# ooowedyn/InkLayer

Hardware: AMD Instinct MI355X
Metric: sketches/sec end-to-end (GroundingDINO+SAM) at 1024x1024 (higher is better)
Workload: dtype f16 (MFMA, f32 accumulate; f32 residual/norm/softmax; split-f16 = fp32-grade operands for patch-embed, neck, mask decoder)

## Files before the change

include/inklayer_hip.h:

```cpp
#ifndef INKLAYER_HIP_H
#define INKLAYER_HIP_H

#include <stdint.h>

#ifdef __cplusplus
extern "C" {
#endif

#define INK_ABI_VERSION 7
int ink_abi_version(void);

typedef struct InkGemm {
  const void* A;
  const void* W;
  const float* bias;
  const float* col_scale;
  const float* residual;
  const int32_t* row_map;
  void* C;
  int32_t M, N, K;
  int32_t lda, ldw, ldr, ldc;
  int32_t act;
  int32_t c_f16;
} InkGemm;
// ... 111 lines not shown

int ink_biattn_fusion(const void* QV_f16, const void* KL_f16, int32_t B, int32_t S, int32_t T, int32_t E,
                      float scale, float* scores_ws, float* stats_ws, float* partial_ws, int32_t chunk,
                      void* out_v_f16, void* out_l_f16, void* stream);

int ink_attn_fewkeys(const void* Q, int64_t ldq, const void* K, int64_t ldk, const void* V, int64_t ldv,
                     int32_t B, int32_t n_q, int32_t n_k, int32_t n_heads, int32_t head_dim, float scale,
                     const uint8_t* blocked, const int32_t* q_batch_rows, const float* q_add, int32_t io_f32, void* O,
                     int64_t ldo, void* stream);

int ink_attn_fewq(const void* Q, int64_t ldq, const void* K, int64_t ldk, const void* V, int64_t ldv,
                  int32_t n_batch, int32_t n_q, int32_t n_k, int32_t n_heads, int32_t head_dim, float scale,
                  const int32_t* q_batch_rows, const int32_t* kv_batch_rows, const float* k_add, int32_t io_f32, void* O,
                  int64_t ldo, void* stream);

int ink_biattn_colstats(const float* scores, int32_t B, int32_t S, int32_t HT, float* part_ws, float* stats, void* stream);

int ink_fusion_fold_workspace(int32_t B, int32_t S, int64_t* out_floats);
int ink_fusion_fold(float* v_f32, int32_t B, int32_t S, const float* lnv_g, const float* lnv_b, float eps,
                    const float* text_k_f32, const float* text_vl_f32, int64_t ld_text, int32_t T, const void* Wq_f16,
                    const float* bq, const void* Wvv_f16, const float* bvv, const void* Wo_f16, const float* bo,
                    const float* gamma_v, float scale, float* ws, void* out_l_f16, const float* pos, void* out16_pos,
                    void* out16, void* stream);

int ink_sam_upscale_pack(const void* ws_f16, void* blob_f16, void* stream);
int ink_sam_upscale_tail(const float* u0, int64_t ld_tok, int32_t n, int32_t g, const float* ln_g, const float* ln_b, float eps,
                         const void* blob_f16, const float* b3, const float* hyper, int32_t n_masks, float* low,
                         void* stream);

int ink_proj256_ln_pack(const void* ws_f16, void* blob_f16, void* stream);
int ink_proj256_ln(const float* a_f32, const void* blob_f16, const float* bias, const float* res_f32,
                   const int32_t* res_batch_rows, int32_t rows_per_batch, const float* ln_g, const float* ln_b, float eps,
                   int64_t rows, float* out_f32, void* out_split_f16, void* stream);

int ink_ffn256_pack_bytes(int32_t hid, int32_t with_pre, int64_t* out_bytes);
int ink_ffn256_pack(const void* w1_f16, const float* b1, const void* w2_f16, int32_t hid, const void* wpre_f16, void* blob,
                    void* stream);
int ink_ffn256_fused(const void* x_f16, int64_t ldx, const float* res_f32, const void* blob, const float* b2,
                     const float* ln_g, const float* ln_b, float eps, int32_t M, int32_t hid, const float* pre_bias,
                     const float* pre_ln_g, const float* pre_ln_b, float* out_f32, void* stream);

int ink_topk_rowmax(const float* logits, int32_t B, int32_t S, int32_t T, int32_t K, int32_t* out_idx,
                    float* out_val, void* cand_ws, void* stream);

int ink_sine_embed4(const float* ref, const float* dim_t, int32_t N, void* out_f16, void* stream);

int ink_box_refine(const float* delta, int64_t ldd, const float* ref, int32_t N, int32_t ref_is_logit,
                   float* out, void* stream);

int ink_mask_cleanup_workspace_ints(int32_t n, int32_t H, int32_t W, int32_t k, int64_t* out_ints);
int ink_mask_cleanup(const void* masks_u8, int32_t n, int32_t H, int32_t W, int32_t k, int32_t area_threshold,
                     double aspect_threshold, void* tmp_a_u8, void* tmp_b_u8, int32_t* workspace, void* out_u8,
                     void* stream);

int ink_mask_sketch_iou_counts(const void* masks_u8, const void* sketch_rgb_u8, int32_t n, int32_t H, int32_t W,
                               void* bits_ws_u64, int32_t* counts, void* stream);

int ink_sam_amg_stats(const float* low, int32_t n, const int32_t* index, int32_t m, const int32_t* m_dev, int32_t S,
                      int32_t L, int32_t in_h, int32_t in_w, int32_t crop_h, int32_t crop_w, double thr, double offset,
                      int32_t x0, int32_t y0, int32_t orig_h, int32_t orig_w, int32_t* table, void* planes_u64,
                      float* out_logits, void* stream);

int ink_mask_rle_counts(const void* planes_u64, const int32_t* select, int32_t k, int32_t H, int32_t W,
                        int32_t* n_counts, void* stream);
int ink_mask_rle_write(const void* planes_u64, const int32_t* select, int32_t k, int32_t H, int32_t W,
                       const int32_t* offsets, int32_t* counts, void* stream);
// ... 54 lines not shown
```

inklayer_amd/_lib.py:

```python
from __future__ import annotations

import ctypes as C
import os
from pathlib import Path

_LIB_PATH = Path(__file__).resolve().parent / "lib" / "libinklayer_hip.so"
_lib = None

c_void_p, c_int, c_i64, c_float = C.c_void_p, C.c_int32, C.c_int64, C.c_float


class InkGemm(C.Structure):
    _fields_ = [
        ("A", c_void_p), ("W", c_void_p), ("bias", c_void_p), ("col_scale", c_void_p),
        ("residual", c_void_p), ("row_map", c_void_p), ("C", c_void_p),
        ("M", c_int), ("N", c_int), ("K", c_int),
        ("lda", c_int), ("ldw", c_int), ("ldr", c_int), ("ldc", c_int),
        ("act", c_int), ("c_f16", c_int),
    ]


class InkAttn(C.Structure):
    _fields_ = [
        ("Q", c_void_p), ("K", c_void_p), ("V", c_void_p), ("O", c_void_p),
# ... 33 lines not shown
                            c_void_p, c_void_p, c_void_p],
    "ink_sam_amg_stats": [c_void_p, c_int, c_void_p, c_int, c_void_p, c_int, c_int, c_int, c_int, c_int, c_int, C.c_double,
                          C.c_double, c_int, c_int, c_int, c_int, c_void_p, c_void_p, c_void_p, c_void_p],
    "ink_mask_rle_counts": [c_void_p, c_void_p, c_int, c_int, c_int, c_void_p, c_void_p],
    "ink_mask_rle_write": [c_void_p, c_void_p, c_int, c_int, c_int, c_void_p, c_void_p, c_void_p],
    "ink_mask_small_regions_workspace_ints": [c_int, c_int, c_int, C.POINTER(c_i64)],
    "ink_mask_small_regions": [c_void_p, c_int, c_int, c_int, c_int, c_int, c_void_p, c_void_p, c_void_p, c_void_p,
                               c_void_p],
    "ink_box_nms": [c_void_p, c_void_p, c_int, c_float, c_void_p, c_void_p, c_void_p, c_void_p],
    "ink_ms_deform_attn_forward": [c_void_p, C.POINTER(c_i64), C.POINTER(c_i64), c_void_p, c_void_p, c_int,
                                   c_int, c_int, c_int, c_int, c_int, c_int, c_int, c_void_p, c_void_p],
    "ink_ms_deform_attn_forward_dev": [c_void_p, c_void_p, c_void_p, c_void_p, c_void_p, c_int, c_int, c_int, c_int,
                                       c_int, c_int, c_int, c_int, c_int, c_void_p, c_void_p],
    "ink_ms_deform_attn_backward_dev": [c_void_p, c_void_p, c_void_p, c_void_p, c_void_p, c_void_p, c_int, c_int, c_int,
                                        c_int, c_int, c_int, c_int, c_int, c_int, c_void_p, c_void_p, c_void_p,
                                        c_void_p],
    "ink_msda_fused": [c_void_p, c_void_p, c_i64, c_void_p, c_int, c_i64, c_i64, C.POINTER(c_int), c_int,
                       c_int, c_int, c_void_p, c_void_p],
    "ink_swin_patchify": [c_void_p, c_int, c_int, C.POINTER(c_float), C.POINTER(c_float), c_void_p, c_void_p],
    "ink_layernorm_merge4": [c_void_p, c_i64, c_void_p, c_void_p, c_float, c_void_p, c_int, c_int, c_void_p,
                             c_void_p],
    "ink_groupnorm_nhwc": [c_void_p, c_int, c_int, c_int, c_int, c_void_p, c_void_p, c_float, c_void_p,
                           c_void_p, c_i64, c_void_p],
    "ink_gather_rows": [c_void_p, c_i64, c_i64, c_void_p, c_i64, c_int, c_int, c_int, c_void_p, c_void_p,
                        c_void_p],
    "ink_biattn_fusion": [c_void_p, c_void_p, c_int, c_int, c_int, c_int, c_float, c_void_p, c_void_p,
                          c_void_p, c_int, c_void_p, c_void_p, c_void_p],
    "ink_biattn_colstats": [c_void_p, c_int, c_int, c_int, c_void_p, c_void_p, c_void_p],
    "ink_fusion_fold_workspace": [c_int, c_int, C.POINTER(c_i64)],
    "ink_relpos_bias64_f16": [c_void_p, c_i64, c_void_p, c_void_p, c_int, c_int, c_int, c_float, c_void_p, c_void_p, c_void_p],
    "ink_proj256_ln_pack": [c_void_p, c_void_p, c_void_p],
    "ink_proj256_ln": [c_void_p, c_void_p, c_void_p, c_void_p, c_void_p, c_int, c_void_p, c_void_p, c_float, c_i64, c_void_p,
                       c_void_p, c_void_p],
    "ink_sam_upscale_pack": [c_void_p, c_void_p, c_void_p],
    "ink_sam_upscale_tail": [c_void_p, c_i64, c_int, c_int, c_void_p, c_void_p, c_float, c_void_p, c_void_p, c_void_p,
                             c_int, c_void_p, c_void_p],
    "ink_ffn256_pack_bytes": [c_int, c_int, C.POINTER(c_i64)],
    "ink_ffn256_pack": [c_void_p, c_void_p, c_void_p, c_int, c_void_p, c_void_p, c_void_p],
    "ink_ffn256_fused": [c_void_p, c_i64, c_void_p, c_void_p, c_void_p, c_void_p, c_void_p, c_float, c_int, c_int,
                         c_void_p, c_void_p, c_void_p, c_void_p, c_void_p],
    "ink_fusion_fold": [c_void_p, c_int, c_int, c_void_p, c_void_p, c_float, c_void_p, c_void_p, c_i64, c_int, c_void_p,
                        c_void_p, c_void_p, c_void_p, c_void_p, c_void_p, c_void_p, c_float, c_void_p, c_void_p, c_void_p,
                        c_void_p, c_void_p, c_void_p],
    "ink_attn_fewkeys": [c_void_p, c_i64, c_void_p, c_i64, c_void_p, c_i64, c_int, c_int, c_int, c_int, c_int,
                         c_float, c_void_p, c_void_p, c_void_p, c_int, c_void_p, c_i64, c_void_p],
    "ink_attn_fewq": [c_void_p, c_i64, c_void_p, c_i64, c_void_p, c_i64, c_int, c_int, c_int, c_int, c_int,
                      c_float, c_void_p, c_void_p, c_void_p, c_int, c_void_p, c_i64, c_void_p],
    "ink_topk_rowmax": [c_void_p, c_int, c_int, c_int, c_int, c_void_p, c_void_p, c_void_p, c_void_p],
    "ink_sine_embed4": [c_void_p, c_void_p, c_int, c_void_p, c_void_p],
    "ink_box_refine": [c_void_p, c_i64, c_void_p, c_int, c_int, c_void_p, c_void_p],
    "ink_mask_cleanup_workspace_ints": [c_int, c_int, c_int, c_int, C.POINTER(c_i64)],
    "ink_mask_cleanup": [c_void_p, c_int, c_int, c_int, c_int, c_int, C.c_double, c_void_p, c_void_p, c_void_p,
                         c_void_p, c_void_p],
    "ink_mask_sketch_iou_counts": [c_void_p, c_void_p, c_int, c_int, c_int, c_void_p, c_void_p, c_void_p],
    "ink_refine_sketch_planes": [c_void_p, c_int, c_int, c_void_p, c_void_p, c_void_p],
    "ink_bitplane_pack": [c_void_p, c_int, c_int, c_int, c_int, c_void_p, c_void_p],
    "ink_refine_depth_samples": [c_void_p, c_int, c_void_p, c_void_p, c_int, c_int, c_int, c_void_p, c_void_p, c_void_p],
    "ink_refine_pair_tables": [c_void_p, c_void_p, c_int, c_int, c_int, c_void_p, c_void_p, c_void_p, c_void_p,
                               c_void_p, c_void_p],
    "ink_refine_composite": [c_void_p, c_void_p, c_int, c_int, c_int, c_void_p, c_void_p, c_void_p],
    "ink_refine_relabel_clean": [c_void_p, c_void_p, c_int, c_int, c_void_p, c_void_p],
    "ink_refine_grow_workspace": [c_int, c_int, C.POINTER(c_i64), C.POINTER(c_i64)],
    "ink_refine_grow": [c_void_p, c_void_p, c_int, c_int, c_void_p, c_void_p, c_void_p, c_void_p, c_void_p, c_void_p,
                        c_int, c_void_p, c_void_p],
    "ink_refine_query_dists": [c_void_p, c_void_p, c_void_p, c_int, c_int, c_int, c_void_p, c_void_p],
    "ink_refine_finalize": [c_void_p, c_void_p, c_int, c_void_p, c_int, c_int, c_void_p, c_void_p, c_void_p, c_void_p],
# ... 44 lines not shown
```

inklayer_amd/csrc/proj_ln.hip:

```cpp
#include <type_traits>
#include "common.h"
#include "../../include/inklayer_hip.h"

namespace {

typedef __attribute__((address_space(1))) const void* gptr_t;
typedef __attribute__((address_space(3))) void* lptr_t;
typedef __attribute__((address_space(3))) char* lds_char_ptr;

constexpr int CI = 128, C = 256, BM = 128;
constexpr int BLK = 1024;
constexpr int NSEG = 3, KSEG = CI / 16;
constexpr int NBLK = (C / 32) * KSEG;
constexpr int CHUNK = NBLK * BLK;
constexpr int PAR_BYTES = 3 * C * 4;
constexpr int OROW = C * 4 + 16;
constexpr int PAR_OFF = 4 * 32 * OROW;
constexpr int LDS_BYTES = PAR_OFF + PAR_BYTES;
constexpr int DEPTH = 4;
static_assert(PAR_OFF >= 2 * CHUNK && LDS_BYTES <= 160 * 1024, "LDS layout");

template <int I> using ic = std::integral_constant<int, I>;
template <int I, int N, class F>
__device__ __forceinline__ void static_for(F&& f) {
  if constexpr (I < N) {
    f(ic<I>{});
    static_for<I + 1, N>(f);
  }
}
__device__ __forceinline__ f32x16 mfma32(const f16x8& a, const f16x8& b, const f32x16& c) {
  return __builtin_amdgcn_mfma_f32_32x32x16_f16(a, b, c, 0, 0, 0);
}
template <int OFF>
__device__ __forceinline__ f16x8 lds_frag(uint32_t addr) {
  f16x8 v;
  asm volatile("ds_read_b128 %0, %1 offset:%2" : "=v"(v) : "v"(addr), "n"(OFF));
  return v;
}
template <int N>
__device__ __forceinline__ void wait_frag(f16x8& f) {
  asm volatile("s_waitcnt lgkmcnt(%1)" : "+v"(f) : "n"(N));
}
template <int OFF>
__device__ __forceinline__ f32x4 lds_f4(uint32_t addr) {
  f32x4 v;
  asm volatile("ds_read_b128 %0, %1 offset:%2" : "=v"(v) : "v"(addr), "n"(OFF));
  return v;
}
__device__ __forceinline__ void wait_f4(f32x4& a, f32x4& b, f32x4& c, f32x4& d) {
  asm volatile("s_waitcnt lgkmcnt(0)" : "+v"(a), "+v"(b), "+v"(c), "+v"(d));
}

__global__ __launch_bounds__(256) void proj_ln_pack_kernel(const f16* __restrict__ ws, f16* __restrict__ blob) {
  const int idx = blockIdx.x * 256 + threadIdx.x;
  if (idx >= NSEG * NBLK * 64) return;
  const int lane = idx & 63, q = (idx >> 6) % NBLK, seg = (idx >> 6) / NBLK;
  const int nt = q / KSEG, s = KSEG * seg + q % KSEG;
  *(f16x8*)(blob + (int64_t)idx * 8) = *(const f16x8*)(ws + (int64_t)(32 * nt + (lane & 31)) * (NSEG * CI) + 16 * s + 8 * (lane >> 5));
}

__global__ __launch_bounds__(256) void proj256_ln_kernel(const float* __restrict__ A, const f16* __restrict__ blob,
                                                         const float* __restrict__ bias, const float* __restrict__ res,
                                                         const int32_t* __restrict__ res_batch_rows, int rows_per_batch,
                                                         const float* __restrict__ ln_g, const float* __restrict__ ln_b,
                                                         float eps, int64_t R, float* __restrict__ out_f32,
                                                         f16* __restrict__ out_split) {
  extern __shared__ __attribute__((aligned(16))) char smem[];
  const int tid = threadIdx.x, lane = tid & 63;
  const int wave = __builtin_amdgcn_readfirstlane(tid >> 6);
  const int l = lane & 31, hh = lane >> 5;
  const int64_t m0 = (int64_t)blockIdx.x * BM + wave * 32;
  const int64_t row = min(m0 + l, R - 1);
  {
    float* sP = (float*)(smem + PAR_OFF);
    sP[tid] = bias[tid];
    sP[C + tid] = ln_g[tid];
    sP[2 * C + tid] = ln_b[tid];
  }
  f16x8 xf[NSEG * KSEG];
  {
    const float* ap = A + row * CI + 8 * hh;
#pragma unroll
    for (int s = 0; s < KSEG; ++s) {
      const f32x4 a0 = *(const f32x4*)(ap + 16 * s), a1 = *(const f32x4*)(ap + 16 * s + 4);
#pragma unroll
      for (int e = 0; e < 8; ++e) {
        const float v = e < 4 ? a0[e] : a1[e - 4];
        const f16 hi = (f16)v;
        xf[s][e] = hi;
        xf[KSEG + s][e] = (f16)((v - (float)hi) * 64.0f);
        xf[2 * KSEG + s][e] = (f16)((float)hi * 0.015625f);
      }
    }
  }
  f32x16 y[C / 32];
  {
    int64_t rrow = row;
    if (res_batch_rows) {
      const int64_t b = row / rows_per_batch;
      rrow = (int64_t)res_batch_rows[b] + (row - b * rows_per_batch);
    }
    const float* rp = res + rrow * C + 4 * hh;
#pragma unroll
    for (int nt = 0; nt < C / 32; ++nt)
#pragma unroll
      for (int g = 0; g < 4; ++g) {
        const f32x4 r4 = *(const f32x4*)(rp + 32 * nt + 8 * g);
#pragma unroll
        for (int e = 0; e < 4; ++e) y[nt][4 * g + e] = r4[e];
      }
// ... 34 lines not shown

  static_for<0, C / 32>([&](auto ii) {
    constexpr int nt = decltype(ii)::value;
    constexpr int ob = (32 * nt) * 4;
    f32x4 c0 = lds_f4<ob>(par0), c1 = lds_f4<ob + 32>(par0), c2 = lds_f4<ob + 64>(par0), c3 = lds_f4<ob + 96>(par0);
    wait_f4(c0, c1, c2, c3);
#pragma unroll
    for (int e = 0; e < 4; ++e) {
      y[nt][e] += c0[e];
      y[nt][4 + e] += c1[e];
      y[nt][8 + e] += c2[e];
      y[nt][12 + e] += c3[e];
    }
  });
  float sum = 0.f;
#pragma unroll
  for (int nt = 0; nt < C / 32; ++nt)
#pragma unroll
    for (int r = 0; r < 16; ++r) sum += y[nt][r];
  sum += __shfl_xor(sum, 32, 64);
  const float mean = sum * (1.0f / C);
  float sq = 0.f;
#pragma unroll
  for (int nt = 0; nt < C / 32; ++nt)
#pragma unroll
    for (int r = 0; r < 16; ++r) {
      const float d = y[nt][r] - mean;
      sq += d * d;
    }
  sq += __shfl_xor(sq, 32, 64);
  const float rstd = 1.0f / sqrtf(sq * (1.0f / C) + eps);
  __syncthreads();
  char* ot = smem + wave * 32 * OROW;
  static_for<0, C / 32 * 2>([&](auto ii) {
    constexpr int nt = decltype(ii)::value / 2, g = 2 * (decltype(ii)::value % 2);
    constexpr int o0 = C * 4 + (32 * nt + 8 * g) * 4;
    f32x4 g0 = lds_f4<o0>(par0), g1 = lds_f4<o0 + 32>(par0), b0 = lds_f4<C * 4 + o0>(par0), b1 = lds_f4<C * 4 + o0 + 32>(par0);
    wait_f4(g0, g1, b0, b1);
    f32x4 v0, v1;
#pragma unroll
    for (int e = 0; e < 4; ++e) {
      v0[e] = (y[nt][4 * g + e] - mean) * rstd * g0[e] + b0[e];
      v1[e] = (y[nt][4 * g + 4 + e] - mean) * rstd * g1[e] + b1[e];
    }
    *(f32x4*)(ot + l * OROW + (32 * nt + 8 * g + 4 * hh) * 4) = v0;
    *(f32x4*)(ot + l * OROW + (32 * nt + 8 * g + 8 + 4 * hh) * 4) = v1;
  });
#pragma unroll 2
  for (int r = 0; r < 32; ++r) {
    const int64_t m = m0 + r;
    if (m >= R) break;
    const f32x4 v = *(const f32x4*)(ot + r * OROW + lane * 16);
    if (out_f32) *(f32x4*)(out_f32 + m * C + lane * 4) = v;
    if (out_split) {
      f16x4 hi, lo, hs;
#pragma unroll
      for (int e = 0; e < 4; ++e) {
        hi[e] = (f16)v[e];
        lo[e] = (f16)((v[e] - (float)hi[e]) * 64.0f);
        hs[e] = (f16)((float)hi[e] * 0.015625f);
      }
      f16* o = out_split + m * (3 * C) + lane * 4;
      *(f16x4*)o = hi;
      *(f16x4*)(o + C) = lo;
      *(f16x4*)(o + 2 * C) = hs;
    }
  }
}

}

extern "C" int ink_proj256_ln_pack(const void* ws_f16, void* blob_f16, void* stream) {
  INK_CHECK_ARG(ws_f16 && blob_f16 && ((((uintptr_t)ws_f16 | (uintptr_t)blob_f16) & 15) == 0));
  hipLaunchKernelGGL(proj_ln_pack_kernel, dim3((NSEG * NBLK * 64 + 255) / 256), dim3(256), 0, (hipStream_t)stream,
                     (const f16*)ws_f16, (f16*)blob_f16);
  return ink_launch_status();
}

extern "C" int ink_proj256_ln(const float* a_f32, const void* blob_f16, const float* bias, const float* res_f32,
                              const int32_t* res_batch_rows, int32_t rows_per_batch, const float* ln_g, const float* ln_b,
                              float eps, int64_t rows, float* out_f32, void* out_split_f16, void* stream) {
  INK_CHECK_ARG(a_f32 && blob_f16 && bias && res_f32 && ln_g && ln_b && rows > 0 && (out_f32 || out_split_f16));
  INK_CHECK_ARG(!res_batch_rows || (rows_per_batch > 0 && rows % rows_per_batch == 0));
  INK_CHECK_ARG((((uintptr_t)a_f32 | (uintptr_t)blob_f16 | (uintptr_t)res_f32 | (uintptr_t)out_f32 |
                  (uintptr_t)out_split_f16) & 15) == 0);
  static bool attr = ((void)hipFuncSetAttribute((const void*)proj256_ln_kernel, hipFuncAttributeMaxDynamicSharedMemorySize,
                                                LDS_BYTES), true);
  (void)attr;
  const int64_t ntiles = (rows + BM - 1) / BM;
  INK_CHECK_ARG(ntiles < (int64_t)1 << 31);
  hipLaunchKernelGGL(proj256_ln_kernel, dim3((unsigned)ntiles), dim3(256), LDS_BYTES, (hipStream_t)stream, a_f32,
                     (const f16*)blob_f16, bias, res_f32, res_batch_rows, rows_per_batch, ln_g, ln_b, eps, rows, out_f32,
                     (f16*)out_split_f16);
  return ink_launch_status();
}
```

inklayer_amd/ops.py:

```python
from __future__ import annotations

import ctypes as C
from typing import Optional, Sequence, Tuple

import torch

from . import _lib
from ._lib import InkAttn, InkGemm, check

ACT = {None: 0, "none": 0, "gelu": 1, "relu": 2}
F16, F32 = torch.float16, torch.float32


_GEMM_TRACE = None


def set_gemm_trace(lst) -> None:
    global _GEMM_TRACE
    _GEMM_TRACE = lst


_ATTN_TRACE = None


# ... 690 lines not shown


def fusion_fold(v: torch.Tensor, B: int, S: int, lnv_g: torch.Tensor, lnv_b: torch.Tensor, eps: float,
                text_kv: torch.Tensor, T: int, Wqv: torch.Tensor, bqv: torch.Tensor, Wo: torch.Tensor, bo: torch.Tensor,
                gamma_v: torch.Tensor, scale: float, pos: Optional[torch.Tensor] = None,
                out16_pos: Optional[torch.Tensor] = None, out16: Optional[torch.Tensor] = None) -> torch.Tensor:
    for t in (out16, out16_pos):
        assert t is None or (t.dtype == F16 and t.is_contiguous() and tuple(t.shape) == (B * S, 256))
    assert out16_pos is None or (pos is not None and pos.dtype == F32 and pos.is_contiguous() and tuple(pos.shape) == (S, 256))
    assert v.dtype == F32 and v.is_contiguous() and tuple(v.shape) == (B * S, 256)
    assert text_kv.dtype == F32 and text_kv.stride(1) == 1 and tuple(text_kv.shape) == (B * T, 2048)
    assert Wqv.dtype == F16 and Wqv.is_contiguous() and tuple(Wqv.shape) == (2048, 256) and bqv.dtype == F32
    assert Wo.dtype == F16 and Wo.is_contiguous() and tuple(Wo.shape) == (256, 1024)
    need = C.c_int64(0)
    check(_lib.lib().ink_fusion_fold_workspace(B, S, C.byref(need)), "ink_fusion_fold_workspace")
    ws = torch.empty(need.value, device=v.device, dtype=F32)
    out_l = torch.empty((B * T, 1024), device=v.device, dtype=F16)
    check(_lib.lib().ink_fusion_fold(v.data_ptr(), B, S, lnv_g.data_ptr(), lnv_b.data_ptr(), eps, text_kv.data_ptr(),
                                     text_kv[:, 1024:].data_ptr(), text_kv.stride(0), T, Wqv.data_ptr(), bqv.data_ptr(),
                                     Wqv[1024:].data_ptr(), bqv[1024:].data_ptr(), Wo.data_ptr(), bo.data_ptr(),
                                     gamma_v.data_ptr(), scale, ws.data_ptr(), out_l.data_ptr(), _p(pos), _p(out16_pos),
                                     _p(out16), _stream()),
          "ink_fusion_fold")
    return out_l


def proj256_ln_pack(ws: torch.Tensor) -> torch.Tensor:
    assert ws.dtype == F16 and ws.is_contiguous() and tuple(ws.shape) == (256, 384)
    blob = torch.empty(3 * 64 * 64 * 8, device=ws.device, dtype=F16)
    check(_lib.lib().ink_proj256_ln_pack(ws.data_ptr(), blob.data_ptr(), _stream()), "ink_proj256_ln_pack")
    return blob


def proj256_ln(a: torch.Tensor, blob: torch.Tensor, bias: torch.Tensor, res: torch.Tensor, ln_g: torch.Tensor,
               ln_b: torch.Tensor, eps: float, *, res_batch_rows: Optional[torch.Tensor] = None, rows_per_batch: int = 0,
               want_f32: bool = True, want_split: bool = True):
    R = int(a.shape[0])
    assert a.dtype == F32 and a.is_contiguous() and tuple(a.shape) == (R, 128)
    assert blob.dtype == F16 and blob.numel() == 3 * 64 * 64 * 8
    assert res.dtype == F32 and res.is_contiguous() and res.shape[1] == 256
    assert all(t.dtype == F32 and t.is_contiguous() and t.numel() == 256 for t in (bias, ln_g, ln_b))
    if res_batch_rows is not None:
        assert res_batch_rows.dtype == torch.int32 and res_batch_rows.is_cuda and rows_per_batch > 0
        assert res_batch_rows.numel() * rows_per_batch == R
    else:
        assert res.shape[0] == R
    of = torch.empty((R, 256), device=a.device, dtype=F32) if want_f32 else None
    osp = torch.empty((R, 768), device=a.device, dtype=F16) if want_split else None
    check(_lib.lib().ink_proj256_ln(a.data_ptr(), blob.data_ptr(), bias.data_ptr(), res.data_ptr(), _p(res_batch_rows),
                                    rows_per_batch, ln_g.data_ptr(), ln_b.data_ptr(), eps, R, _p(of), _p(osp), _stream()),
          "ink_proj256_ln")
    return of, osp


def sam_upscale_pack(ws: torch.Tensor) -> torch.Tensor:
    assert ws.dtype == F16 and ws.is_contiguous() and tuple(ws.shape) == (128, 192)
    blob = torch.empty(4 * 12 * 64 * 8, device=ws.device, dtype=F16)
    check(_lib.lib().ink_sam_upscale_pack(ws.data_ptr(), blob.data_ptr(), _stream()), "ink_sam_upscale_pack")
    return blob


def sam_upscale_tail(u0: torch.Tensor, n: int, g: int, ln_g: torch.Tensor, ln_b: torch.Tensor, eps: float,
                     blob: torch.Tensor, b3: torch.Tensor, hyper: torch.Tensor) -> torch.Tensor:
    if u0.shape[1] == 64:
        assert u0.is_contiguous() and u0.shape[0] == n * g * g * 4
        u0 = u0.view(n * g * g, 256)
    assert u0.dtype == F32 and u0.stride(1) == 1 and tuple(u0.shape) == (n * g * g, 256) and u0.stride(0) % 4 == 0
    assert blob.dtype == F16 and blob.numel() == 4 * 12 * 64 * 8 and b3.dtype == F32 and b3.numel() == 128
    assert hyper.dtype == F32 and hyper.is_contiguous() and hyper.dim() == 3 and hyper.shape[0] == n and hyper.shape[2] == 32
    assert ln_g.dtype == F32 and ln_b.dtype == F32 and ln_g.numel() == 64 and ln_b.numel() == 64
    M = hyper.shape[1]
    low = torch.empty((n, M, 4 * g, 4 * g), device=u0.device, dtype=F32)
    check(_lib.lib().ink_sam_upscale_tail(_p(u0), u0.stride(0), n, g, _p(ln_g), _p(ln_b), eps, _p(blob), _p(b3), _p(hyper), M,
                                          _p(low), _stream()), "ink_sam_upscale_tail")
    return low


def ffn256_pack(w1: torch.Tensor, b1: torch.Tensor, w2: torch.Tensor, w_pre: Optional[torch.Tensor] = None) -> torch.Tensor:
    hid = int(w1.shape[0])
    assert w1.dtype == F16 and w2.dtype == F16 and w1.is_contiguous() and w2.is_contiguous()
# ... 173 lines not shown
```

inklayer_amd/sam.py:

```python
from __future__ import annotations

import math
from dataclasses import dataclass
from typing import Dict, List, Optional, Sequence, Tuple

import numpy as np
import torch

from . import ops
from ._lru import LRU

F16, F32 = torch.float16, torch.float32


@dataclass
class SamConfig:
    embed_dim: int = 1280
    depth: int = 32
    num_heads: int = 16
    global_attn_indexes: Tuple[int, ...] = (7, 15, 23, 31)
    window_size: int = 14
    img_size: int = 1024
    patch_size: int = 16
    mlp_ratio: float = 4.0
# ... 190 lines not shown
                .to(dev).contiguous()
        ar = (torch.arange(g, dtype=torch.float32) + 0.5) / g
        grid_xy = torch.stack([ar[None, :].expand(g, g), ar[:, None].expand(g, g)], -1).reshape(-1, 2)
        self.dense_pe = ops.sam_pe_encode(grid_xy.contiguous().to(dev), w["gauss"])

        t = "mask_decoder.transformer."
        def attn(dst, src):
            for n in ("q_proj", "k_proj", "v_proj", "out_proj"):
                w[f"{dst}.{n}.ws"] = ws(f"{src}.{n}.weight")
                w[f"{dst}.{n}.b"] = f(f"{src}.{n}.bias")

        def cat(dst, names):
            for sfx in (".ws", ".b"):
                w[dst + sfx] = torch.cat([w[n + sfx] for n in names]).contiguous()

        pe_split = ops.add_split_f16(self.dense_pe)
        for i in range(cfg.dec_depth):
            p, d = f"{t}layers.{i}.", f"d{i}"
            attn(d + ".self", p + "self_attn")
            attn(d + ".t2i", p + "cross_attn_token_to_image")
            attn(d + ".i2t", p + "cross_attn_image_to_token")
            if i == 0:
                cat(d + ".self.qkv", [f"{d}.self.{n}" for n in ("q_proj", "k_proj", "v_proj")])
            else:
                cat(d + ".self.qk", [f"{d}.self.{n}" for n in ("q_proj", "k_proj")])
            for n in ("norm1", "norm2", "norm3", "norm4"):
                w[f"{d}.{n}.w"], w[f"{d}.{n}.b"] = f(p + n + ".weight"), f(p + n + ".bias")
            w[d + ".lin1.ws"], w[d + ".lin1.b"] = ws(p + "mlp.lin1.weight"), f(p + "mlp.lin1.bias")
            w[d + ".lin2.ws"], w[d + ".lin2.b"] = ws(p + "mlp.lin2.weight"), f(p + "mlp.lin2.bias")
            cat(d + ".kvq", [d + ".t2i.k_proj", d + ".t2i.v_proj", d + ".i2t.q_proj"])
            w[d + ".t2i.k_pe"] = ops.gemm(pe_split, w[d + ".t2i.k_proj.ws"]).contiguous()
            w[d + ".i2t.q_pe"] = ops.gemm(pe_split, w[d + ".i2t.q_proj.ws"]).contiguous()
            w[d + ".i2t.out_proj.blob"] = ops.proj256_ln_pack(w[d + ".i2t.out_proj.ws"].contiguous())
        attn("dfin", t + "final_attn_token_to_image")
        w["dfin.norm.w"], w["dfin.norm.b"] = f(t + "norm_final_attn.weight"), f(t + "norm_final_attn.bias")
        w["dfin.k_pe"] = ops.gemm(pe_split, w["dfin.k_proj.ws"]).contiguous()
        w["out_tok"] = torch.cat([f("mask_decoder.iou_token.weight"),
                                  f("mask_decoder.mask_tokens.weight")], 0).contiguous()
        u = "mask_decoder.output_upscaling."
        w["up0.ws"] = ws(u + "0.weight", lambda t: t.permute(2, 3, 1, 0).reshape(4 * (E // 4), E))
        w["up0.b"] = f(u + "0.bias").repeat(4).contiguous()
        w["up1.w"], w["up1.b"] = f(u + "1.weight"), f(u + "1.bias")
        up3 = ws(u + "3.weight", lambda t: t.permute(2, 3, 1, 0).reshape(4 * (E // 8), E // 4))
        assert tuple(up3.shape) == (128, 192)
        w["up3.blob"] = ops.sam_upscale_pack(up3.contiguous())
        w["up3.b"] = f(u + "3.bias").repeat(4).contiguous()
        cat("dfin.kvu", ["dfin.k_proj", "dfin.v_proj", "up0"])
        for j in range(3):
            w[f"iou{j}.ws"] = ws(f"mask_decoder.iou_prediction_head.layers.{j}.weight")
            w[f"iou{j}.b"] = f(f"mask_decoder.iou_prediction_head.layers.{j}.bias")
            for m in range(cfg.num_mask_tokens):
                hk = f"mask_decoder.output_hypernetworks_mlps.{m}.layers.{j}."
                if m == 0 or hk + "bias" in sd:
                    w[f"{_hyp(m)}{j}.b"] = f(hk + "bias")
                if m == 0 or hk + "weight" in sd:
                    w[f"{_hyp(m)}{j}.ws"] = ws(hk + "weight")

        self._alloc(max_batch)
        if bias_correction:
            self._calibrate_bias_correction(sd)

    @torch.no_grad()
    def _calibrate_bias_correction(self, sd) -> None:
        cfg, w, D = self.cfg, self.w, self.cfg.embed_dim
        page = torch.full((cfg.img_size, cfg.img_size, 3), 255, dtype=torch.uint8, device=self.dev)
        means: Dict[str, torch.Tensor] = {}
        self._calib = means
        try:
            self.encode([page])
        finally:
            self._calib = None
        for i in range(cfg.depth):
            p = f"image_encoder.blocks.{i}."
            for lin in ("attn.qkv", "mlp.lin1", "attn.proj", "mlp.lin2"):
                W32 = sd[p + lin + ".weight"].detach().to(self.dev, torch.float32)
                w16, bkey = w[f"b{i}.{lin}.weight"], f"b{i}.{lin}.bias"
                w[bkey] = (w[bkey].double() + (W32 - w16.float()).double() @ means[f"b{i}.{lin}"].double()).float().contiguous()

    def _alloc(self, B: int) -> None:
        cfg, dev, T, D = self.cfg, self.dev, self.T, self.cfg.embed_dim
# ... 170 lines not shown
        img_rows = _to_dev_async((iob * T).to(torch.int32), dev)
        if mask_input is None:
            keys = ops.add_f32(emb.reshape(B * T, E).contiguous(), w["no_mask"])
            shared = True
            ks = None
        else:
            keys, ks = ops.sam_mask_embed(mask_input, emb.reshape(B * T, E).contiguous(), img_rows, w["mask_ds"], 1e-6,
                                          split=True)
            shared = False
        queries = qpe
        sc32, sc16 = 1.0 / math.sqrt(32), 1.0 / math.sqrt(16)

        Eh = E // 2

        def t2i_attend(name, queries, k, v, k_pe, residual):
            q = lin(SP(queries, qpe), name + ".q_proj")
            a = ops.attn_fewq(q, k, v, n_batch=n, n_heads=Hh, head_dim=16, scale=sc16, n_q=NT, n_k=T,
                              kv_batch_rows=img_rows if shared else None, k_add=k_pe)
            return lin(SP(a), name + ".out_proj", residual=residual)

        for i in range(cfg.dec_depth):
            d = f"d{i}"
            if i == 0:
                qkv = ops.gemm(SP(queries), w[d + ".self.qkv.ws"], w[d + ".self.qkv.b"])
                a = ops.attn_fewkeys(qkv[:, :E], qkv[:, E:2 * E], qkv[:, 2 * E:], B=n, n_heads=Hh, head_dim=32,
                                     scale=sc32)
                queries = lin(SP(a), d + ".self.out_proj")
            else:
                qk = ops.gemm(SP(queries, qpe), w[d + ".self.qk.ws"], w[d + ".self.qk.b"])
                v = lin(SP(queries), d + ".self.v_proj")
                a = ops.attn_fewkeys(qk[:, :E], qk[:, E:], v, B=n, n_heads=Hh, head_dim=32, scale=sc32)
                queries = lin(SP(a), d + ".self.out_proj", residual=queries)
            queries = ops.layernorm_rows(queries, w[d + ".norm1.w"], w[d + ".norm1.b"], 1e-5, out_dtype=F32)
            kvq = ops.gemm(SP(keys) if ks is None else ks, w[d + ".kvq.ws"], w[d + ".kvq.b"])
            queries = ops.layernorm_rows(t2i_attend(d + ".t2i", queries, kvq[:, :Eh], kvq[:, Eh:2 * Eh],
                                                    w[d + ".t2i.k_pe"], queries),
                                         w[d + ".norm2.w"], w[d + ".norm2.b"], 1e-5, out_dtype=F32)
            hmid = lin(SP(queries), d + ".lin1", act="relu")
            queries = ops.layernorm_rows(lin(SP(hmid), d + ".lin2", residual=queries),
                                         w[d + ".norm3.w"], w[d + ".norm3.b"], 1e-5, out_dtype=F32)
            ik = lin(SP(queries, qpe), d + ".i2t.k_proj")
            iv = lin(SP(queries), d + ".i2t.v_proj")
            a = ops.attn_fewkeys(kvq[:, 2 * Eh:], ik, iv, B=n, n_heads=Hh, head_dim=16, scale=sc16, n_q=T,
                                 q_batch_rows=img_rows if shared else None, q_add=w[d + ".i2t.q_pe"])
            last = i + 1 == cfg.dec_depth
            keys, ks = ops.proj256_ln(a, w[d + ".i2t.out_proj.blob"], w[d + ".i2t.out_proj.b"], keys, w[d + ".norm4.w"],
                                      w[d + ".norm4.b"], 1e-5, res_batch_rows=img_rows if shared else None,
                                      rows_per_batch=T if shared else 0, want_f32=not last, want_split=True)
            shared = False
        kvu = ops.gemm(ks, w["dfin.kvu.ws"], w["dfin.kvu.b"])
        kv = kvu[:, :2 * Eh]
        queries = ops.layernorm_rows(t2i_attend("dfin", queries, kv[:, :Eh], kv[:, Eh:], w["dfin.k_pe"], queries),
                                     w["dfin.norm.w"], w["dfin.norm.b"], 1e-5, out_dtype=F32)
        hs = queries.view(n, NT, E)

        def mlp3(prefix: str, x: torch.Tensor) -> torch.Tensor:
            a = lin(SP(x), prefix + "0", act="relu")
            a = lin(SP(a), prefix + "1", act="relu")
            return lin(SP(a), prefix + "2")

        M = n_masks
        if M == 1:
            hyper = mlp3(_hyp(mask_lo), hs[:, 1 + mask_lo].contiguous()).view(n, 1, 32)
        else:
            hyper = torch.stack([mlp3(_hyp(m), hs[:, 1 + m].contiguous()) for m in range(mask_lo, mask_lo + M)], 1)
        iou = mlp3("iou", hs[:, 0].contiguous())[:, mask_lo:mask_lo + M]
        u0 = kvu[:, 2 * Eh:]
        low = ops.sam_upscale_tail(u0, n, g, w["up1.w"], w["up1.b"], 1e-6, w["up3.blob"], w["up3.b"], hyper)
        return low, iou


class SamPredictor:

    def __init__(self, engine: SamEngine):
        self.engine = engine
        self.cfg = engine.cfg
        self.transform = ResizeLongestSide(engine.cfg.img_size)
        self.reset_image()

    def reset_image(self) -> None:
        self.is_image_set = False
        self.features = None
        self.original_size = None
# ... 91 lines not shown
```

Baseline: 118.2.

## Fuse next layer's KVQ projection into proj256+LayerNorm kernel epilogue

Extends the proj256_ln kernel with a templated epilogue that takes the normalized rows, forms split-f16 operands in registers, and runs the next decoder layer's kvq (or final kvu) GEMM against a pre-packed weight blob. This removes the split-f16 round trip to global memory and a separate GEMM launch per decoder layer. The cost is more register and LDS pressure in the fused kernel, extra pack kernels at load time, and a specialised weight layout for N=384/512.

Result: no change. 118.5, median of 6 (+0.3%).

```diff
diff --git a/include/inklayer_hip.h b/include/inklayer_hip.h
--- a/include/inklayer_hip.h
+++ b/include/inklayer_hip.h
@@ -167,6 +167,12 @@
 int ink_proj256_ln(const float* a_f32, const void* blob_f16, const float* bias, const float* res_f32,
                    const int32_t* res_batch_rows, int32_t rows_per_batch, const float* ln_g, const float* ln_b, float eps,
                    int64_t rows, float* out_f32, void* out_split_f16, void* stream);
+int ink_proj256_ln_next_pack_bytes(int32_t next_n, int64_t* out_bytes);
+int ink_proj256_ln_next_pack(const void* ws_f16, int32_t next_n, void* blob_f16, void* stream);
+int ink_proj256_ln_next(const float* a_f32, const void* blob_f16, const float* bias, const float* res_f32,
+                        const int32_t* res_batch_rows, int32_t rows_per_batch, const float* ln_g, const float* ln_b,
+                        float eps, int64_t rows, float* out_f32, const void* next_blob_f16, const float* next_bias,
+                        int32_t next_n, float* next_out, int64_t next_ld, void* stream);
 
 int ink_ffn256_pack_bytes(int32_t hid, int32_t with_pre, int64_t* out_bytes);
 int ink_ffn256_pack(const void* w1_f16, const float* b1, const void* w2_f16, int32_t hid, const void* wpre_f16, void* blob,
diff --git a/inklayer_amd/_lib.py b/inklayer_amd/_lib.py
--- a/inklayer_amd/_lib.py
+++ b/inklayer_amd/_lib.py
@@ -89,6 +89,10 @@
     "ink_proj256_ln_pack": [c_void_p, c_void_p, c_void_p],
     "ink_proj256_ln": [c_void_p, c_void_p, c_void_p, c_void_p, c_void_p, c_int, c_void_p, c_void_p, c_float, c_i64, c_void_p,
                        c_void_p, c_void_p],
+    "ink_proj256_ln_next_pack_bytes": [c_int, C.POINTER(c_i64)],
+    "ink_proj256_ln_next_pack": [c_void_p, c_int, c_void_p, c_void_p],
+    "ink_proj256_ln_next": [c_void_p, c_void_p, c_void_p, c_void_p, c_void_p, c_int, c_void_p, c_void_p, c_float, c_i64,
+                            c_void_p, c_void_p, c_void_p, c_int, c_void_p, c_i64, c_void_p],
     "ink_sam_upscale_pack": [c_void_p, c_void_p, c_void_p],
     "ink_sam_upscale_tail": [c_void_p, c_i64, c_int, c_int, c_void_p, c_void_p, c_float, c_void_p, c_void_p, c_void_p,
                              c_int, c_void_p, c_void_p],
diff --git a/inklayer_amd/csrc/proj_ln.hip b/inklayer_amd/csrc/proj_ln.hip
--- a/inklayer_amd/csrc/proj_ln.hip
+++ b/inklayer_amd/csrc/proj_ln.hip
@@ -18,7 +18,13 @@
 constexpr int PAR_OFF = 4 * 32 * OROW;
 constexpr int LDS_BYTES = PAR_OFF + PAR_BYTES;
 constexpr int DEPTH = 4;
-static_assert(PAR_OFF >= 2 * CHUNK && LDS_BYTES <= 160 * 1024, "LDS layout");
+constexpr int NMAX = 512;
+constexpr int KN = NSEG * C / 16;
+constexpr int PASS_CHUNKS = 8 * KN / NBLK;
+constexpr int LDS_BYTES_NEXT = LDS_BYTES + NMAX * 4;
+static_assert(PAR_OFF >= 2 * CHUNK && LDS_BYTES_NEXT <= 160 * 1024, "LDS layout");
+
+__host__ __device__ constexpr int next_perm(int p) { return (p & 7) < 4 ? 4 * (p >> 3) + (p & 7) : 8 + 4 * (p >> 3) + (p & 7) - 4; }
 
 template <int I> using ic = std::integral_constant<int, I>;
 template <int I, int N, class F>
@@ -59,12 +65,29 @@
   *(f16x8*)(blob + (int64_t)idx * 8) = *(const f16x8*)(ws + (int64_t)(32 * nt + (lane & 31)) * (NSEG * CI) + 16 * s + 8 * (lane >> 5));
 }
 
+__global__ __launch_bounds__(256) void proj_ln_next_pack_kernel(const f16* __restrict__ ws, f16* __restrict__ blob, int N) {
+  const int idx = blockIdx.x * 256 + threadIdx.x;
+  if (idx >= (N / 32) * KN * 64) return;
+  const int lane = idx & 63, q = (idx >> 6) % NBLK, gc = (idx >> 6) / NBLK;
+  const int pass = gc >= PASS_CHUNKS, c = gc - PASS_CHUNKS * pass;
+  const int kpc = (pass && N == 384) ? 16 : 8;
+  const int nt = q / kpc, s = kpc * c + q % kpc;
+  const f16* src = ws + (int64_t)(256 * pass + 32 * nt + (lane & 31)) * (NSEG * C) + 16 * s;
+  f16x8 v;
+#pragma unroll
+  for (int e = 0; e < 8; ++e) v[e] = src[next_perm(8 * (lane >> 5) + e)];
+  *(f16x8*)(blob + (int64_t)idx * 8) = v;
+}
+
+template <int NN>
 __global__ __launch_bounds__(256) void proj256_ln_kernel(const float* __restrict__ A, const f16* __restrict__ blob,
                                                          const float* __restrict__ bias, const float* __restrict__ res,
                                                          const int32_t* __restrict__ res_batch_rows, int rows_per_batch,
                                                          const float* __restrict__ ln_g, const float* __restrict__ ln_b,
                                                          float eps, int64_t R, float* __restrict__ out_f32,
-                                                         f16* __restrict__ out_split) {
+                                                         f16* __restrict__ out_split, const f16* __restrict__ nblob,
+                                                         const float* __restrict__ nbias, float* __restrict__ nout,
+                                                         int64_t nld) {
   extern __shared__ __attribute__((aligned(16))) char smem[];
   const int tid = threadIdx.x, lane = tid & 63;
   const int wave = __builtin_amdgcn_readfirstlane(tid >> 6);
@@ -76,6 +99,10 @@
     sP[tid] = bias[tid];
     sP[C + tid] = ln_g[tid];
     sP[2 * C + tid] = ln_b[tid];
+    if constexpr (NN > 0) {
+      sP[3 * C + tid] = nbias[tid];
+      if (C + tid < NN) sP[4 * C + tid] = nbias[C + tid];
+    }
   }
   f16x8 xf[NSEG * KSEG];
   {
@@ -176,39 +203,143 @@
   const float rstd = 1.0f / sqrtf(sq * (1.0f / C) + eps);
   __syncthreads();
   char* ot = smem + wave * 32 * OROW;
-  static_for<0, C / 32 * 2>([&](auto ii) {
-    constexpr int nt = decltype(ii)::value / 2, g = 2 * (decltype(ii)::value % 2);
-    constexpr int o0 = C * 4 + (32 * nt + 8 * g) * 4;
-    f32x4 g0 = lds_f4<o0>(par0), g1 = lds_f4<o0 + 32>(par0), b0 = lds_f4<C * 4 + o0>(par0), b1 = lds_f4<C * 4 + o0 + 32>(par0);
-    wait_f4(g0, g1, b0, b1);
-    f32x4 v0, v1;
-#pragma unroll
-    for (int e = 0; e < 4; ++e) {
-      v0[e] = (y[nt][4 * g + e] - mean) * rstd * g0[e] + b0[e];
-      v1[e] = (y[nt][4 * g + 4 + e] - mean) * rstd * g1[e] + b1[e];
-    }
-    *(f32x4*)(ot + l * OROW + (32 * nt + 8 * g + 4 * hh) * 4) = v0;
-    *(f32x4*)(ot + l * OROW + (32 * nt + 8 * g + 8 + 4 * hh) * 4) = v1;
-  });
+  if constexpr (NN == 0) {
+    static_for<0, C / 32 * 2>([&](auto ii) {
+      constexpr int nt = decltype(ii)::value / 2, g = 2 * (decltype(ii)::value % 2);
+      constexpr int o0 = C * 4 + (32 * nt + 8 * g) * 4;
+      f32x4 g0 = lds_f4<o0>(par0), g1 = lds_f4<o0 + 32>(par0), b0 = lds_f4<C * 4 + o0>(par0), b1 = lds_f4<C * 4 + o0 + 32>(par0);
+      wait_f4(g0, g1, b0, b1);
+      f32x4 v0, v1;
+#pragma unroll
+      for (int e = 0; e < 4; ++e) {
+        v0[e] = (y[nt][4 * g + e] - mean) * rstd * g0[e] + b0[e];
+        v1[e] = (y[nt][4 * g + 4 + e] - mean) * rstd * g1[e] + b1[e];
+      }
+      *(f32x4*)(ot + l * OROW + (32 * nt + 8 * g + 4 * hh) * 4) = v0;
+      *(f32x4*)(ot + l * OROW + (32 * nt + 8 * g + 8 + 4 * hh) * 4) = v1;
+    });
 #pragma unroll 2
-  for (int r = 0; r < 32; ++r) {
-    const int64_t m = m0 + r;
-    if (m >= R) break;
-    const f32x4 v = *(const f32x4*)(ot + r * OROW + lane * 16);
-    if (out_f32) *(f32x4*)(out_f32 + m * C + lane * 4) = v;
-    if (out_split) {
-      f16x4 hi, lo, hs;
+    for (int r = 0; r < 32; ++r) {
+      const int64_t m = m0 + r;
+      if (m >= R) break;
+      const f32x4 v = *(const f32x4*)(ot + r * OROW + lane * 16);
+      if (out_f32) *(f32x4*)(out_f32 + m * C + lane * 4) = v;
+      if (out_split) {
+        f16x4 hi, lo, hs;
+#pragma unroll
+        for (int e = 0; e < 4; ++e) {
+          hi[e] = (f16)v[e];
+          lo[e] = (f16)((v[e] - (float)hi[e]) * 64.0f);
+          hs[e] = (f16)((float)hi[e] * 0.015625f);
+        }
+        f16* o = out_split + m * (3 * C) + lane * 4;
+        *(f16x4*)o = hi;
+        *(f16x4*)(o + C) = lo;
+        *(f16x4*)(o + 2 * C) = hs;
+      }
+    }
+  } else {
+    f16x8 xn[KN];
+    static_for<0, C / 32 * 2>([&](auto ii) {
+      constexpr int s = decltype(ii)::value, nt = s / 2, g = 2 * (s % 2);
+      constexpr int o0 = C * 4 + (32 * nt + 8 * g) * 4;
+      f32x4 g0 = lds_f4<o0>(par0), g1 = lds_f4<o0 + 32>(par0), b0 = lds_f4<C * 4 + o0>(par0), b1 = lds_f4<C * 4 + o0 + 32>(par0);
+      wait_f4(g0, g1, b0, b1);
+      f32x4 v0, v1;
 #pragma unroll
       for (int e = 0; e < 4; ++e) {
-        hi[e] = (f16)v[e];
-        lo[e] = (f16)((v[e] - (float)hi[e]) * 64.0f);
-        hs[e] = (f16)((float)hi[e] * 0.015625f);
-      }
-      f16* o = out_split + m * (3 * C) + lane * 4;
-      *(f16x4*)o = hi;
-      *(f16x4*)(o + C) = lo;
-      *(f16x4*)(o + 2 * C) = hs;
-    }
+        v0[e] = (y[nt][4 * g + e] - mean) * rstd * g0[e] + b0[e];
+        v1[e] = (y[nt][4 * g + 4 + e] - mean) * rstd * g1[e] + b1[e];
+      }
+#pragma unroll
+      for (int e = 0; e < 8; ++e) {
+        const float v = e < 4 ? v0[e] : v1[e - 4];
+        const f16 hi = (f16)v;
+        xn[s][e] = hi;
+        xn[C / 16 + s][e] = (f16)((v - (float)hi) * 64.0f);
+        xn[2 * (C / 16) + s][e] = (f16)((float)hi * 0.015625f);
+      }
+      if (out_f32) {
+        *(f32x4*)(ot + l * OROW + (32 * nt + 8 * g + 4 * hh) * 4) = v0;
+        *(f32x4*)(ot + l * OROW + (32 * nt + 8 * g + 8 + 4 * hh) * 4) = v1;
+      }
+    });
+    if (out_f32) {
+#pragma unroll 2
+      for (int r = 0; r < 32; ++r) {
+        const int64_t m = m0 + r;
+        if (m >= R) break;
+        *(f32x4*)(out_f32 + m * C + lane * 4) = *(const f32x4*)(ot + r * OROW + lane * 16);
+      }
+    }
+
+    auto nstage = [&](int buf, int gc, int k) {
+      const int q = 4 * k + wave;
+      __builtin_amdgcn_global_load_lds((gptr_t)((const char*)nblob + (int64_t)gc * CHUNK + q * BLK + lane * 16),
+                                       (lptr_t)(smem + buf * CHUNK + q * BLK), 16, 0, 0);
+    };
+    auto pass = [&](auto ntp_c, auto gc0_c, auto col0_c) {
+      constexpr int NTP = decltype(ntp_c)::value, GC0 = decltype(gc0_c)::value, COL0 = decltype(col0_c)::value;
+      constexpr int NCH = NTP * KN / NBLK, KPC = NBLK / NTP;
+      asm volatile("s_waitcnt lgkmcnt(0)" ::: "memory");
+      __builtin_amdgcn_s_barrier();
+      asm volatile("" ::: "memory");
+#pragma unroll
+      for (int k = 0; k < NBLK / 4; ++k) nstage(0, GC0, k);
+      f32x16 acc[NTP];
+      static_for<0, NTP>([&](auto ii) {
+        constexpr int nt = decltype(ii)::value;
+        constexpr int ob = 3 * C * 4 + (COL0 + 32 * nt) * 4;
+        f32x4 c0 = lds_f4<ob>(par0), c1 = lds_f4<ob + 32>(par0), c2 = lds_f4<ob + 64>(par0), c3 = lds_f4<ob + 96>(par0);
+        wait_f4(c0, c1, c2, c3);
+#pragma unroll
+        for (int e = 0; e < 4; ++e) {
+          acc[nt][e] = c0[e];
+          acc[nt][4 + e] = c1[e];
+          acc[nt][8 + e] = c2[e];
+          acc[nt][12 + e] = c3[e];
+        }
+      });
+      static_for<0, NCH>([&](auto cc) {
+        constexpr int c = decltype(cc)::value;
+        asm volatile("s_waitcnt vmcnt(0)" ::: "memory");
+        __builtin_amdgcn_s_barrier();
+        asm volatile("" ::: "memory");
+        const uint32_t wa = lds0 + (c & 1) * CHUNK;
+        f16x8 fr[DEPTH + 1];
+        auto read = [&](auto ii) {
+          constexpr int i = decltype(ii)::value;
+          fr[i % (DEPTH + 1)] = lds_frag<i * BLK>(wa);
+        };
+        static_for<0, DEPTH>(read);
+        static_for<0, NBLK>([&](auto ii) {
+          constexpr int i = decltype(ii)::value;
+          if constexpr (i + DEPTH < NBLK) read(ic<i + DEPTH>{});
+          wait_frag<(NBLK - 1 - i < DEPTH ? NBLK - 1 - i : DEPTH)>(fr[i % (DEPTH + 1)]);
+          acc[i / KPC] = mfma32(fr[i % (DEPTH + 1)], xn[KPC * c + i % KPC], acc[i / KPC]);
+          if constexpr (c + 1 < NCH && i % 4 == 1) nstage((c + 1) & 1, GC0 + c + 1, i / 4);
+        });
+      });
+      __syncthreads();
+      static_for<0, NTP * 4>([&](auto ii) {
+        constexpr int nt = decltype(ii)::value / 4, g = decltype(ii)::value % 4;
+        f32x4 v;
+#pragma unroll
+        for (int e = 0; e < 4; ++e) v[e] = acc[nt][4 * g + e];
+        *(f32x4*)(ot + l * OROW + (32 * nt + 8 * g + 4 * hh) * 4) = v;
+      });
+      constexpr int LPR = 8 * NTP, RPI = 64 / LPR;
+#pragma unroll 2
+      for (int r0 = 0; r0 < 32; r0 += RPI) {
+        const int r = r0 + lane / LPR;
+        const int64_t m = m0 + r;
+        if (m0 + r0 >= R) break;
+        const f32x4 v = *(const f32x4*)(ot + r * OROW + (lane % LPR) * 16);
+        if (m < R) *(f32x4*)(nout + m * nld + COL0 + (lane % LPR) * 4) = v;
+      }
+    };
+    pass(ic<8>{}, ic<0>{}, ic<0>{});
+    pass(ic<(NN - 256) / 32>{}, ic<PASS_CHUNKS>{}, ic<256>{});
   }
 }
 
@@ -219,6 +350,38 @@
   hipLaunchKernelGGL(proj_ln_pack_kernel, dim3((NSEG * NBLK * 64 + 255) / 256), dim3(256), 0, (hipStream_t)stream,
                      (const f16*)ws_f16, (f16*)blob_f16);
   return ink_launch_status();
+}
+
+extern "C" int ink_proj256_ln_next_pack_bytes(int32_t n, int64_t* out_bytes) {
+  INK_CHECK_ARG(out_bytes && (n == 384 || n == 512));
+  *out_bytes = (int64_t)n * NSEG * C * 2;
+  return INK_OK;
+}
+
+extern "C" int ink_proj256_ln_next_pack(const void* ws_f16, int32_t n, void* blob_f16, void* stream) {
+  INK_CHECK_ARG(ws_f16 && blob_f16 && ((((uintptr_t)ws_f16 | (uintptr_t)blob_f16) & 15) == 0) && (n == 384 || n == 512));
+  hipLaunchKernelGGL(proj_ln_next_pack_kernel, dim3(((n / 32) * KN * 64 + 255) / 256), dim3(256), 0, (hipStream_t)stream,
+                     (const f16*)ws_f16, (f16*)blob_f16, n);
+  return ink_launch_status();
+}
+
+namespace {
+template <int NN>
+int launch_proj256_ln(const float* a_f32, const void* blob_f16, const float* bias, const float* res_f32,
+                      const int32_t* res_batch_rows, int32_t rows_per_batch, const float* ln_g, const float* ln_b, float eps,
+                      int64_t rows, float* out_f32, void* out_split_f16, const void* next_blob_f16, const float* next_bias,
+                      float* next_out, int64_t next_ld, void* stream) {
+  constexpr int lds = NN ? LDS_BYTES_NEXT : LDS_BYTES;
+  static bool attr = ((void)hipFuncSetAttribute((const void*)proj256_ln_kernel<NN>,
+                                                hipFuncAttributeMaxDynamicSharedMemorySize, lds), true);
+  (void)attr;
+  const int64_t ntiles = (rows + BM - 1) / BM;
+  INK_CHECK_ARG(ntiles < (int64_t)1 << 31);
+  hipLaunchKernelGGL(proj256_ln_kernel<NN>, dim3((unsigned)ntiles), dim3(256), lds, (hipStream_t)stream, a_f32,
+                     (const f16*)blob_f16, bias, res_f32, res_batch_rows, rows_per_batch, ln_g, ln_b, eps, rows, out_f32,
+                     (f16*)out_split_f16, (const f16*)next_blob_f16, next_bias, next_out, next_ld);
+  return ink_launch_status();
+}
 }
 
 extern "C" int ink_proj256_ln(const float* a_f32, const void* blob_f16, const float* bias, const float* res_f32,
@@ -228,13 +391,20 @@
   INK_CHECK_ARG(!res_batch_rows || (rows_per_batch > 0 && rows % rows_per_batch == 0));
   INK_CHECK_ARG((((uintptr_t)a_f32 | (uintptr_t)blob_f16 | (uintptr_t)res_f32 | (uintptr_t)out_f32 |
                   (uintptr_t)out_split_f16) & 15) == 0);
-  static bool attr = ((void)hipFuncSetAttribute((const void*)proj256_ln_kernel, hipFuncAttributeMaxDynamicSharedMemorySize,
-                                                LDS_BYTES), true);
-  (void)attr;
-  const int64_t ntiles = (rows + BM - 1) / BM;
-  INK_CHECK_ARG(ntiles < (int64_t)1 << 31);
-  hipLaunchKernelGGL(proj256_ln_kernel, dim3((unsigned)ntiles), dim3(256), LDS_BYTES, (hipStream_t)stream, a_f32,
-                     (const f16*)blob_f16, bias, res_f32, res_batch_rows, rows_per_batch, ln_g, ln_b, eps, rows, out_f32,
-                     (f16*)out_split_f16);
-  return ink_launch_status();
-}
+  return launch_proj256_ln<0>(a_f32, blob_f16, bias, res_f32, res_batch_rows, rows_per_batch, ln_g, ln_b, eps, rows, out_f32,
+                              out_split_f16, nullptr, nullptr, nullptr, 0, stream);
+}
+
+extern "C" int ink_proj256_ln_next(const float* a_f32, const void* blob_f16, const float* bias, const float* res_f32,
+                                   const int32_t* res_batch_rows, int32_t rows_per_batch, const float* ln_g,
+                                   const float* ln_b, float eps, int64_t rows, float* out_f32, const void* next_blob_f16,
+                                   const float* next_bias, int32_t next_n, float* next_out, int64_t next_ld, void* stream) {
+  INK_CHECK_ARG(a_f32 && blob_f16 && bias && res_f32 && ln_g && ln_b && rows > 0 && next_blob_f16 && next_bias && next_out);
+  INK_CHECK_ARG(!res_batch_rows || (rows_per_batch > 0 && rows % rows_per_batch == 0));
+  INK_CHECK_ARG((next_n == 384 || next_n == 512) && next_ld >= next_n && next_ld % 4 == 0);
+  INK_CHECK_ARG((((uintptr_t)a_f32 | (uintptr_t)blob_f16 | (uintptr_t)res_f32 | (uintptr_t)out_f32 |
+                  (uintptr_t)next_blob_f16 | (uintptr_t)next_bias | (uintptr_t)next_out) & 15) == 0);
+  auto go = next_n == 384 ? launch_proj256_ln<384> : launch_proj256_ln<512>;
+  return go(a_f32, blob_f16, bias, res_f32, res_batch_rows, rows_per_batch, ln_g, ln_b, eps, rows, out_f32, nullptr,
+            next_blob_f16, next_bias, next_out, next_ld, stream);
+}
diff --git a/inklayer_amd/ops.py b/inklayer_amd/ops.py
--- a/inklayer_amd/ops.py
+++ b/inklayer_amd/ops.py
@@ -746,9 +746,20 @@
     return blob
 
 
+def proj256_ln_next_pack(ws: torch.Tensor) -> torch.Tensor:
+    N = int(ws.shape[0])
+    assert ws.dtype == F16 and ws.is_contiguous() and tuple(ws.shape) == (N, 768)
+    need = C.c_int64(0)
+    check(_lib.lib().ink_proj256_ln_next_pack_bytes(N, C.byref(need)), "ink_proj256_ln_next_pack_bytes")
+    blob = torch.empty(need.value // 2, device=ws.device, dtype=F16)
+    check(_lib.lib().ink_proj256_ln_next_pack(ws.data_ptr(), N, blob.data_ptr(), _stream()), "ink_proj256_ln_next_pack")
+    return blob
+
+
 def proj256_ln(a: torch.Tensor, blob: torch.Tensor, bias: torch.Tensor, res: torch.Tensor, ln_g: torch.Tensor,
                ln_b: torch.Tensor, eps: float, *, res_batch_rows: Optional[torch.Tensor] = None, rows_per_batch: int = 0,
-               want_f32: bool = True, want_split: bool = True):
+               want_f32: bool = True, want_split: bool = True, next_blob: Optional[torch.Tensor] = None,
+               next_bias: Optional[torch.Tensor] = None, next_n: int = 0, next_out: Optional[torch.Tensor] = None):
     R = int(a.shape[0])
     assert a.dtype == F32 and a.is_contiguous() and tuple(a.shape) == (R, 128)
     assert blob.dtype == F16 and blob.numel() == 3 * 64 * 64 * 8
@@ -760,6 +771,18 @@
     else:
         assert res.shape[0] == R
     of = torch.empty((R, 256), device=a.device, dtype=F32) if want_f32 else None
+    if next_blob is not None:
+        assert next_n in (384, 512) and next_blob.dtype == F16 and next_blob.numel() == next_n * 768
+        assert next_bias is not None and next_bias.dtype == F32 and next_bias.is_contiguous() and next_bias.numel() == next_n
+        if next_out is None:
+            next_out = torch.empty((R, next_n), device=a.device, dtype=F32)
+        assert next_out.dtype == F32 and tuple(next_out.shape) == (R, next_n) and next_out.stride(1) == 1
+        check(_lib.lib().ink_proj256_ln_next(a.data_ptr(), blob.data_ptr(), bias.data_ptr(), res.data_ptr(),
+                                             _p(res_batch_rows), rows_per_batch, ln_g.data_ptr(), ln_b.data_ptr(), eps, R,
+                                             _p(of), next_blob.data_ptr(), next_bias.data_ptr(), next_n,
+                                             next_out.data_ptr(), next_out.stride(0), _stream()), "ink_proj256_ln_next")
+        return of, next_out
+    assert next_bias is None and next_out is None and next_n == 0
     osp = torch.empty((R, 768), device=a.device, dtype=F16) if want_split else None
     check(_lib.lib().ink_proj256_ln(a.data_ptr(), blob.data_ptr(), bias.data_ptr(), res.data_ptr(), _p(res_batch_rows),
                                     rows_per_batch, ln_g.data_ptr(), ln_b.data_ptr(), eps, R, _p(of), _p(osp), _stream()),
diff --git a/inklayer_amd/sam.py b/inklayer_amd/sam.py
--- a/inklayer_amd/sam.py
+++ b/inklayer_amd/sam.py
@@ -246,6 +246,8 @@
             w[d + ".t2i.k_pe"] = ops.gemm(pe_split, w[d + ".t2i.k_proj.ws"]).contiguous()
             w[d + ".i2t.q_pe"] = ops.gemm(pe_split, w[d + ".i2t.q_proj.ws"]).contiguous()
             w[d + ".i2t.out_proj.blob"] = ops.proj256_ln_pack(w[d + ".i2t.out_proj.ws"].contiguous())
+            if i > 0:
+                w[d + ".kvq.blob"] = ops.proj256_ln_next_pack(w[d + ".kvq.ws"])
         attn("dfin", t + "final_attn_token_to_image")
         w["dfin.norm.w"], w["dfin.norm.b"] = f(t + "norm_final_attn.weight"), f(t + "norm_final_attn.bias")
         w["dfin.k_pe"] = ops.gemm(pe_split, w["dfin.k_proj.ws"]).contiguous()
@@ -260,6 +262,7 @@
         w["up3.blob"] = ops.sam_upscale_pack(up3.contiguous())
         w["up3.b"] = f(u + "3.bias").repeat(4).contiguous()
         cat("dfin.kvu", ["dfin.k_proj", "dfin.v_proj", "up0"])
+        w["dfin.kvu.blob"] = ops.proj256_ln_next_pack(w["dfin.kvu.ws"])
         for j in range(3):
             w[f"iou{j}.ws"] = ws(f"mask_decoder.iou_prediction_head.layers.{j}.weight")
             w[f"iou{j}.b"] = f(f"mask_decoder.iou_prediction_head.layers.{j}.bias")
@@ -496,7 +499,8 @@
                 a = ops.attn_fewkeys(qk[:, :E], qk[:, E:], v, B=n, n_heads=Hh, head_dim=32, scale=sc32)
                 queries = lin(SP(a), d + ".self.out_proj", residual=queries)
             queries = ops.layernorm_rows(queries, w[d + ".norm1.w"], w[d + ".norm1.b"], 1e-5, out_dtype=F32)
-            kvq = ops.gemm(SP(keys) if ks is None else ks, w[d + ".kvq.ws"], w[d + ".kvq.b"])
+            if i == 0:
+                kvq = ops.gemm(SP(keys) if ks is None else ks, w[d + ".kvq.ws"], w[d + ".kvq.b"])
             queries = ops.layernorm_rows(t2i_attend(d + ".t2i", queries, kvq[:, :Eh], kvq[:, Eh:2 * Eh],
                                                     w[d + ".t2i.k_pe"], queries),
                                          w[d + ".norm2.w"], w[d + ".norm2.b"], 1e-5, out_dtype=F32)
@@ -508,11 +512,13 @@
             a = ops.attn_fewkeys(kvq[:, 2 * Eh:], ik, iv, B=n, n_heads=Hh, head_dim=16, scale=sc16, n_q=T,
                                  q_batch_rows=img_rows if shared else None, q_add=w[d + ".i2t.q_pe"])
             last = i + 1 == cfg.dec_depth
-            keys, ks = ops.proj256_ln(a, w[d + ".i2t.out_proj.blob"], w[d + ".i2t.out_proj.b"], keys, w[d + ".norm4.w"],
-                                      w[d + ".norm4.b"], 1e-5, res_batch_rows=img_rows if shared else None,
-                                      rows_per_batch=T if shared else 0, want_f32=not last, want_split=True)
+            nxt = "dfin.kvu" if last else f"d{i + 1}.kvq"
+            keys, kvq = ops.proj256_ln(a, w[d + ".i2t.out_proj.blob"], w[d + ".i2t.out_proj.b"], keys, w[d + ".norm4.w"],
+                                       w[d + ".norm4.b"], 1e-5, res_batch_rows=img_rows if shared else None,
+                                       rows_per_batch=T if shared else 0, want_f32=not last,
+                                       next_blob=w[nxt + ".blob"], next_bias=w[nxt + ".b"], next_n=w[nxt + ".b"].numel())
             shared = False
-        kvu = ops.gemm(ks, w["dfin.kvu.ws"], w["dfin.kvu.b"])
+        kvu = kvq
         kv = kvu[:, :2 * Eh]
         queries = ops.layernorm_rows(t2i_attend("dfin", queries, kv[:, :Eh], kv[:, Eh:], w["dfin.k_pe"], queries),
                                      w["dfin.norm.w"], w["dfin.norm.b"], 1e-5, out_dtype=F32)
```
